# NeSC-IV/sage-icp

Measured on AMD Instinct MI355X. Metric: ICP frames/sec (120k-pt scan vs 1M-pt map), higher is better.
Workload: dtype f64

## Files before the change

profiles/loop_tail.py:

```python
import ctypes as C
import os
import sys

sys.path.insert(0, os.getcwd())
import numpy as np
import sage_icp_amd as sage

sage.LIB_PATH = os.environ.get("LOOP_LIB", os.path.join(os.path.dirname(sage.LIB_PATH), "_probe", "libsageicp_looptiming.so"))
from sage_icp_amd import synthetic as syn

div = int(sys.argv[1]) if len(sys.argv) > 1 else 1
p = syn.PARAMS[sys.argv[2] if len(sys.argv) > 2 else "cold"]
name = sys.argv[3] if len(sys.argv) > 3 else "c2"
w = syn.make_workload(name, lambda: sage.VoxelHashMap(syn.WORKLOADS[name]["voxel"], 100.0))
n = len(w["scan"]) // div
f = sage.Frame(w["map"], w["scan"][:n])
os.environ["SAGEICP_LOOP"] = "2"
sage.set_counting(False)
for _ in range(3):
    pose, st = sage.register_frame(f, w["map"], sage.IDENTITY, p["max_dist"], p["kernel"], p["sem_th"], return_stats=True)
assert st.single_launch == 1
IT, WG = 32, 2048
wg = np.zeros((IT, WG, 4), dtype=np.uint64)
sv = np.zeros((IT, 4), dtype=np.uint64)
# ... 46 lines not shown
    print("   %d CUs: " % len(keys) + "; ".join("%d hold %d workgroups (last counted in %.2f)" % ((pop == k).sum(), k, fin[pop[inv] == k].max()) for k in sorted(set(pop))))
    print("   extra units per CU: " + "; ".join("%d CUs with %d (last counted in %.2f)" % ((nx == k).sum(), k, fin[nx[inv] == k].max()) for k in sorted(set(nx))))
    late = np.argsort(-fin)[:10]
    print("   last ten: " + "; ".join("%.1f (%s, %d pts max, %d stale, %d pts, CU pop %d / %d extra)" % (
        fin[o], "extra %.1f-%.1f" % (s2[o], e2[o]) if extra[o] else "no extra", info[it, used, 1][o], info[it, used, 2][o], info[it, used, 3][o],
        pop[inv[o]], nx[inv[o]]) for o in late))

if hasattr(sage.lib(), "sageicp_debug_loop_waves"):
    wv = np.zeros((IT, WG, 8, 2), dtype=np.uint64)
    sage.lib().sageicp_debug_loop_waves(wv.ctypes.data_as(C.c_void_p))
    for it in (12,):
        if it >= min(IT, st.iterations):
            continue
        t0 = sv[it - 1, 3]
        rec = wv[it][used]
        nwv = int((rec[0, :, 0] > 0).sum())
        end = rec[:, :nwv, 0].astype(np.float64) / 100.0 - t0
        meta = rec[:, :nwv, 1]
        start = ((rec[:, :nwv, 0] & ~np.uint64((1 << 40) - 1)) | (meta >> np.uint64(24))).astype(np.float64) / 100.0 - t0
        unit = ((meta >> np.uint64(16)) & np.uint64(0xFF)).astype(int)
        simd = ((meta >> np.uint64(4)) & np.uint64(3)).astype(int)
        slot = (meta & np.uint64(0xF)).astype(int)
        print("iteration %d, first units of the %d waves of a workgroup:" % (it, nwv))
        for k in range(nwv):
            print("   wave %d: SIMD histogram %s | slot histogram %s | unit taken histogram %s | start p50 %.2f | end p10 %.2f p50 %.2f p90 %.2f p100 %.2f"
                  % (k, np.bincount(simd[:, k], minlength=4).tolist(), np.bincount(slot[:, k], minlength=10).tolist(),
                     np.bincount(unit[:, k], minlength=nwv).tolist(), np.median(start[:, k]), q(end[:, k], .1), q(end[:, k], .5), q(end[:, k], .9), end[:, k].max()))
        for u in range(nwv):
            sel = unit == u
            print("   unit %d (by last iteration's work, heaviest first): lasts p10 %.2f p50 %.2f p90 %.2f p100 %.2f | ends p50 %.2f p90 %.2f p100 %.2f"
                  % (u, q((end - start)[sel], .1), q((end - start)[sel], .5), q((end - start)[sel], .9), (end - start)[sel].max(),
                     q(end[sel], .5), q(end[sel], .9), end[sel].max()))
        print("   distinct SIMDs per workgroup: " + str(np.bincount([len(set(r)) for r in simd.tolist()], minlength=5).tolist()))
        xcc = (info[it, used, 0] >> 28).astype(np.int64)
        cu = ((info[it, used, 0] >> 8) & 0xF).astype(np.int64)
        se = ((info[it, used, 0] >> 13) & 0x7).astype(np.int64)
        key = (((xcc << 4 | se) << 4 | cu)[:, None] << 2) | simd
        keys, inv = np.unique(key.ravel(), return_inverse=True)
        heavy = np.zeros(len(keys)); cnt = np.zeros(len(keys)); last = np.zeros(len(keys))
        np.add.at(heavy, inv, (unit.ravel() == 0).astype(float))
        np.add.at(cnt, inv, 1.0)
        np.maximum.at(last, inv, end.ravel())
        print("   %d SIMDs: waves per SIMD histogram %s; heaviest units (unit 0) per SIMD histogram %s" % (len(keys), np.bincount(cnt.astype(int)).tolist(), np.bincount(heavy.astype(int)).tolist()))
        for h in sorted(set(heavy.astype(int))):
            print("      SIMDs with %d heaviest units: %d, last first-unit ends mean %.2f max %.2f" % (h, (heavy == h).sum(), last[heavy == h].mean(), last[heavy == h].max()))
```

sage-icp_amd/csrc/icp_body.h:

```cpp
#pragma once

namespace sageicp {

#ifndef SAGE_LOOP_FLAT_MINW
#define SAGE_LOOP_FLAT_MINW 8
#endif
#ifndef SAGE_SCAN_AHEAD
#define SAGE_SCAN_AHEAD 1
#endif
#ifndef SAGE_ROW_SHIFT_LAYER
#define SAGE_ROW_SHIFT_LAYER 1
#endif
#ifndef SAGE_ROW_SHIFT_MAXW
#define SAGE_ROW_SHIFT_MAXW 4
#endif

struct PairCompact {
    uint4 a, b;
    unsigned ka, oa;
    bool ha, hb;
};
struct PairFull {
    Point4 a, b;
    unsigned ka;
// ... 36 lines not shown
    const double slack = (GIVEN ? fs : 1e-9 * vs) + 1e-13 * fabs(v);
    const double lo = fmax((v - below_hi) - slack, 0.0);
    const double hi = fmax((above_lo - v) - slack, 0.0);
    g[0] = (lo * lo) * sc;
    g[1] = 0.0;
    g[2] = (hi * hi) * sc;
}

__device__ __forceinline__ float round_up_f32(double x) {
    return __uint_as_float(__float_as_uint(static_cast<float>(x)) + 1u);
}

template <int LW>
__device__ __forceinline__ bool reduce_argmin(double best, unsigned bkey, bool valid, const uint32_t *lrow, unsigned &mkey, unsigned &woff) {
    constexpr int W = 1 << LW, SH = 5;
    const double m = seg_min_f64<W>(best);
    const unsigned mine = (best == m) ? bkey : 0xFFFFFFFFu;
    mkey = seg_min_u32<W>(mine);
    const bool found = valid && mkey != 0xFFFFFFFFu;
    woff = (lrow[found ? mkey >> 8 : 0u] >> 8) * (kUnitPoints * 32u) + ((mkey & 255u) << SH);
    return found;
}

template <int LW, bool FUSED, bool FILT, bool PERSIST = false, bool FLATQ = false>
__device__ __forceinline__ void icp_body(const IcpParams &P, uint32_t *smem, LoopGroup *G = nullptr, const double *pose = nullptr) {
    static_assert(!PERSIST || FUSED, "the persistent loop always accumulates");
    constexpr int W = 1 << LW;
    constexpr int QW = 64 >> LW;
    constexpr int SH = 5;
    PROBE_NN_BEGIN(np);
    PROBE_DELAY_BEGIN(t0);
    int lane;
    if constexpr (PERSIST) {
        unsigned l;
        asm volatile("v_mbcnt_lo_u32_b32 %0, -1, 0\n\tv_mbcnt_hi_u32_b32 %0, -1, %0" : "=v"(l));
        lane = static_cast<int>(l);
    } else {
        lane = static_cast<int>(threadIdx.x & 63u);
    }
    const int wv = __builtin_amdgcn_readfirstlane(static_cast<int>(threadIdx.x >> 6));
    if (FUSED && !PERSIST) {
        if (threadIdx.x == 0) {
            smem[kWgArrive] = 0u;
            smem[kWgGo] = 0u;
        }
        if (threadIdx.x < 2u * kWgAccWords) smem[kWgAcc + threadIdx.x] = 0u;
        if (threadIdx.x < 12u && !(P.chain && P.chain_iter > 0))
            reinterpret_cast<double *>(smem + kWgPose)[threadIdx.x] = threadIdx.x < 9u ? P.st->R[threadIdx.x] : P.st->T[4u + threadIdx.x - 9u];
        __syncthreads();
    }
    uint32_t *wl;
    if constexpr (PERSIST) wl = G->rows;
    else wl = smem + kWgHeaderWords + static_cast<unsigned>(wv) * icp_wave_words(LW);

    unsigned wave_id, stripe_id = 0u;
    if constexpr (PERSIST) wave_id = G->slot;
    else wave_id = icp_wave_of_stripe(P, wv, stripe_id);

    const int qw = lane >> LW;
    const unsigned ci = static_cast<unsigned>(lane) & (W - 1u);
    unsigned q, qslot = 0u, bslot = 0u;
    if constexpr (PERSIST) {
        bslot = G->perm[G->unit * (QW / 4) + static_cast<unsigned>(qw >> 2)];
        qslot = bslot * 4u + (static_cast<unsigned>(qw) & 3u);
        q = G->q_first + qslot;
    } else {
        q = wave_id * QW + static_cast<unsigned>(qw);
    }
    const bool valid = q < static_cast<unsigned>(P.n);
    const unsigned qc = valid ? q : 0u;
    uint32_t *lrow = wl + (PERSIST ? qslot : static_cast<unsigned>(qw)) * kRowLdsStride;
    const uint32_t *grow = P.rows + static_cast<size_t>(qc) * kRowWords;

    const __amdgpu_buffer_rsrc_t pts = __builtin_amdgcn_make_buffer_rsrc(
        const_cast<Point4 *>(P.pts), 0, static_cast<int>(P.pts_bytes), 0x00020000);

    const __amdgpu_buffer_rsrc_t cands = __builtin_amdgcn_make_buffer_rsrc(
        const_cast<uint4 *>(P.cand), 0, static_cast<int>(P.cand_bytes), 0x00020000);
    constexpr int SHC = FILT ? 4 : 5;

    constexpr int NP = (7 + W - 1) / W;
    uint4 rk;
    uint2 prev = make_uint2(0xFFFFFFFFu, 0u);
    Point4 f;
    uint4 pc0 = make_uint4(0u, 0u, 0u, 0u), pc1 = pc0, pc2 = pc0, pc3 = pc0, pc4 = pc0, pc5 = pc0, pc6 = pc0;
    uint32_t *lst = nullptr;
    if constexpr (PERSIST) {
        lst = G->state + qslot * kLoopStateWords;
        const uint4 fa = *reinterpret_cast<const uint4 *>(lst), fb = *reinterpret_cast<const uint4 *>(lst + 4);
        const uint4 pk = *reinterpret_cast<const uint4 *>(lst + kStPrev);
        const uint2 ko = *reinterpret_cast<const uint2 *>(lst + kStPrev + 4);
        f.x = __hiloint2double(static_cast<int>(fa.y), static_cast<int>(fa.x));
        f.y = __hiloint2double(static_cast<int>(fa.w), static_cast<int>(fa.z));
        f.z = __hiloint2double(static_cast<int>(fb.y), static_cast<int>(fb.x));
        f.l = __hiloint2double(static_cast<int>(fb.w), static_cast<int>(fb.z));
        prev = make_uint2(pk.x, pk.y);
        rk = make_uint4(pk.z, pk.w, ko.x, ko.y);
    } else {
        rk = *reinterpret_cast<const uint4 *>(grow + kRowKey);
        if (FUSED) prev = P.nn_prev[qc];
        f = P.frame[qc];
        auto row_piece = [&](int k) {
            const unsigned p = min(ci + static_cast<unsigned>(W * k), 6u);
            return *reinterpret_cast<const uint4 *>(grow + 4u * p);
        };
        pc0 = row_piece(0); pc1 = pc0; pc2 = pc0; pc3 = pc0; pc4 = pc0; pc5 = pc0; pc6 = pc0;
        if (NP > 1) pc1 = row_piece(1);
        if (NP > 2) pc2 = row_piece(2);
        if (NP > 3) pc3 = row_piece(3);
        if (NP > 4) pc4 = row_piece(4);
        if (NP > 5) pc5 = row_piece(5);
        if (NP > 6) pc6 = row_piece(6);
    }
    PROBE_DELAY_WAIT(P, t0);
    if constexpr (FUSED && !PERSIST) {
        if (P.chain && P.chain_iter > 0) {
            if (wv == 0) chain_wait_pose(P, smem, lane);
            __syncthreads();
            if (smem[kWgGo]) return;
        }
    }
    const Query s = [&]() {
        if constexpr (PERSIST) {
            return make_query<(W >= 4)>(f, pose, pose + 9, 1, P.voxel_size, P.inv_voxel_size, static_cast<unsigned>(lane));
        } else if constexpr (FUSED) {
            const double *lpose = reinterpret_cast<const double *>(smem + kWgPose);
            return make_query<(W >= 4)>(f, lpose, lpose + 9, P.apply_pose, P.voxel_size, P.inv_voxel_size, threadIdx.x);
        } else {
            return make_query<(W >= 4)>(f, P.st->R, P.st->T + 4, P.apply_pose, P.voxel_size, P.inv_voxel_size, threadIdx.x);
        }
    }();
    const bool stale = valid && (static_cast<uint32_t>(s.kx) != rk.x || static_cast<uint32_t>(s.ky) != rk.y ||
                                 static_cast<uint32_t>(s.kz) != rk.z);
    unsigned occ = rk.w;
    NN_T(np, 0);
    LP_T(PERSIST, G, 0);
    if constexpr (!PERSIST) {
        auto stage = [&](int k, const uint4 &v) {
            const unsigned p = ci + static_cast<unsigned>(W * k);
            if (p < 7u) *reinterpret_cast<uint4 *>(lrow + 4u * p) = v;
        };
        stage(0, pc0);
        if (NP > 1) stage(1, pc1);
        if (NP > 2) stage(2, pc2);
// ... 156 lines not shown
            }
        }
    }
    if constexpr (PERSIST) {
        __builtin_amdgcn_fence(__ATOMIC_ACQ_REL, "wavefront");
        prev.x = lst[opaque_v(kStPrev)];
    }
    if (!valid) occ = 0u;

    double gx[3], gy[3], gz[3];
    {
        const double vs = P.voxel_size, sc = P.prune_scale;
        double fs = 0.0;
        if constexpr (PERSIST) fs = reinterpret_cast<const LoopArgs *>(&P)->face_slack;
        axis_gaps<PERSIST>(s.x, s.kx, vs, sc, fs, gx);
        axis_gaps<PERSIST>(s.y, s.ky, vs, sc, fs, gy);
        axis_gaps<PERSIST>(s.z, s.kz, vs, sc, fs, gz);
    }
    NN_T(np, 1);
    LP_T(PERSIST, G, 1);

    double best = P.dist_init;
    unsigned bkey = 0xFFFFFFFFu;
    const int pli = static_cast<int>(s.l);
    const double th = P.sem_th;
    unsigned npairs = 0u;

    unsigned k = ci, kend = 0u, off = 0u;
    unsigned pk = 0u, needs = 0u, wn = 0u;
    auto evaluate = [&](const Point4 &nb, bool on, unsigned key) {
        const double dx = nb.x - s.x, dy = nb.y - s.y, dz = nb.z - s.z;
        double d = SAGE_SQNORM3_NN(dx * dx, dy * dy, dz * dz);
        const bool same = static_cast<int>(nb.l) == pli || fabs(nb.l * s.l) < 1.0;
        const double ds = d * th;
        d = same ? ds : d;
        d = __hiloint2double(on ? __double2hiint(d) : 0x7FF80000, __double2loint(d));
        const bool lt = d < best, eq = d == best, kl = key < bkey;
        const bool take = lt | (eq & kl);
        best = min_f64(best, d);
        bkey = take ? key : bkey;
    };

    const float qx = static_cast<float>(s.x), qy = static_cast<float>(s.y), qz = static_cast<float>(s.z);
    const float plab = static_cast<float>(pli);
    const bool q_zero = pli == 0;
    bool unknown = false;
    double slack = 0.0;
// ... 177 lines not shown

    constexpr unsigned kHome = 13u;
    bool merged = false;
    if constexpr (PERSIST) {
        const bool seeded = valid && prev.x != 0xFFFFFFFFu;
        const Point4 pp = *reinterpret_cast<const Point4 *>(lst + 8);
        evaluate(pp, seeded, prev.x);
        merged = seeded;
        const unsigned first = seeded ? 0u : (occ & (1u << kHome));
        if (__ballot(first != 0u)) scan(first, nullptr, false, 0u);
    } else if (FUSED) {
        const bool seeded = valid && prev.x != 0xFFFFFFFFu;
        const Point4 pp = load_point(pts, seeded ? prev.y : 0u);
        scan(occ & (1u << kHome), &pp, seeded, prev.x);
    } else {
        scan(occ & (1u << kHome), nullptr, false, 0u);
    }
    NN_T(np, 2);
    LP_T(PERSIST, G, 2);
    const double bound = seg_min_f64<W>(best);
    fb = bound;
    unsigned need = P.keep_all;
    if constexpr (W >= 4) {
        const unsigned a = ci & 3u;
        const double ga = a == 0u ? gx[0] : (a == 2u ? gx[2] : 0.0);
        unsigned layer = 0u;
#pragma unroll
        for (int b = 0; b < 3; ++b) {
#pragma unroll
            for (int c = 0; c < 3; ++c) {
                const double lb = ga + (gy[b] + gz[c]);
                layer |= (lb <= bound) ? (1u << (3 * b + c)) : 0u;
            }
        }
        layer = (a < 3u && ci < 4u) ? layer << (9u * a) : 0u;
        layer |= dpp_u32<kDppXor1>(layer);
        layer |= dpp_u32<kDppXor2>(layer);
        if (W >= 8) layer |= dpp_u32<kDppHalfMirror>(layer);
        if (W >= 16) layer |= dpp_u32<kDppMirror>(layer);
        need |= layer & ~(1u << kHome);
    } else {
#pragma unroll
        for (int v = 0; v < 27; ++v) {
            if (v == static_cast<int>(kHome)) continue;
            const double lb = gx[v / 9] + (gy[(v / 3) % 3] + gz[v % 3]);
            need |= (lb <= bound) ? (1u << v) : 0u;
        }
// ... 129 lines not shown
```

sage-icp_amd/csrc/kernels.hip:

```cpp

#include <hip/hip_runtime.h>

#include <algorithm>
#include <cfloat>
#include <cstdlib>
#include <type_traits>
#include <vector>

#ifndef SAGE_ICP_STRIPE
#define SAGE_ICP_STRIPE 8
#endif
#ifndef SAGE_ICP_OCC
#define SAGE_ICP_OCC 6
#endif

#include "kernels.h"
#include "se3_math.h"
#include "sageicp_types.h"
#include "probes.h"

namespace sageicp {


template <int CTRL>
// ... 330 lines not shown
        {
            if (ok) (void)__hip_atomic_fetch_add(dst + lane, x, __ATOMIC_RELAXED, __HIP_MEMORY_SCOPE_AGENT);
            else (void)__hip_atomic_fetch_or(overflow, 1ll, __ATOMIC_RELAXED, __HIP_MEMORY_SCOPE_AGENT);
        }
    }
}

struct LoopGroup {
    uint32_t *rows;
    uint32_t *state;
    const uint32_t *perm;
    uint32_t *work;
    unsigned unit;
    double *red;
    unsigned long long *wgacc;
    unsigned q_first;
    unsigned slot;
    PROBE_LOOP_GROUP_FIELDS
};
constexpr int kLoopMaxWaves = kLoopMaxWavesHost;
constexpr unsigned kLoopStripe = kLoopStripeHost;
constexpr int kNoVoxel = 0x7FFFFFFF;
constexpr unsigned kStPrev = 16, kStKey = 18;
constexpr unsigned kLpArrive = 0, kLpNext = 1, kLpDone = 2;
constexpr unsigned kLpPose = 4;
constexpr unsigned kLpDbg = kLpPose + 24u;
constexpr unsigned kLpFirst = kLpDbg + 4u;
constexpr unsigned kLpAcc = kLpFirst + 8u;
constexpr unsigned kLpHeaderWords = (kLpAcc + 2u * kWgAccWords + 15u) & ~15u;
__host__ __device__ constexpr unsigned loop_red_words() { return 2u * kCount * 4u; }
__host__ __device__ constexpr unsigned loop_perm_words(unsigned nblk) { return 2u * ((nblk + 7u) & ~7u); }
template <typename W>
struct LoopLds {
    W perm, work, rows, state, red, end;
    __host__ __device__ constexpr LoopLds(int lw, W nw, W gpw)
        : perm(kLpHeaderWords),
          work(perm + loop_perm_words(static_cast<unsigned>(gpw) * ((64u >> lw) / 4u)) / 2u),
          rows(perm + loop_perm_words(static_cast<unsigned>(gpw) * ((64u >> lw) / 4u))),
          state(rows + gpw * static_cast<W>(64 >> lw) * static_cast<W>(kRowLdsStride)),
          red(state + gpw * static_cast<W>(64 >> lw) * static_cast<W>(kLoopStateWords)),
          end(red + nw * loop_red_words()) {}
};

__device__ __forceinline__ unsigned loop_pose_copy(int pose_map, unsigned b = blockIdx.x) {
    return pose_map == 1 ? 0u : ((pose_map == 2 ? b + 3u : b) & static_cast<unsigned>(kLoopPoseCopies - 1));
}
__device__ __forceinline__ void chain_wait_pose(const IcpParams &P, uint32_t *smem, int lane) {
// ... 304 lines not shown
```

sage-icp_amd/csrc/loop_kernel.h:

```cpp
#pragma once

namespace sageicp {


__device__ __forceinline__ int exchange_sums_wave(double *S, const P2pParams &X, unsigned long long g) {
    const int lane = static_cast<int>(threadIdx.x & 63u);
    const int slot = static_cast<int>(g & 1ull);
    const unsigned long long tag = g + 1ull;
    if (lane < kNumSums) {
        const double v = S[lane];
        for (int r = 0; r < X.nranks; ++r)
            __hip_atomic_store(&X.block[r]->sums[slot][X.rank][lane], v, __ATOMIC_RELAXED, __HIP_MEMORY_SCOPE_SYSTEM);
    }
    asm volatile("s_waitcnt vmcnt(0)" ::: "memory");
    __builtin_amdgcn_fence(__ATOMIC_RELEASE, "");
    asm volatile("s_waitcnt vmcnt(0)" ::: "memory");
    if (lane == 0)
        for (int r = 0; r < X.nranks; ++r)
            __hip_atomic_store(&X.block[r]->flag[X.rank], tag, __ATOMIC_RELAXED, __HIP_MEMORY_SCOPE_SYSTEM);
    P2pBlock *mine = X.block[X.rank];
    bool late = false, gone = false;
    if (lane < X.nranks) {
        const unsigned long long t0 = __builtin_amdgcn_s_memrealtime();
        while (__hip_atomic_load(&mine->flag[lane], __ATOMIC_RELAXED, __HIP_MEMORY_SCOPE_SYSTEM) < tag) {
// ... 296 lines not shown
            idx = jb;
            nwg = static_cast<unsigned>(L.wgs) >> 3;
        } else {
            idx = ((jb / kLoopStripe) * 8u + xcd) * kLoopStripe + (jb % kLoopStripe);
            nwg = static_cast<unsigned>(L.wgs);
        }
        const unsigned base = cnt / nwg, extra = cnt - base * nwg;
        g0 = lo + idx * base + min(idx, extra);
        gcnt = min(gpw, base + (idx < extra ? 1u : 0u));
    }
    constexpr unsigned BPW = QW / 4;
    const unsigned nblk_max = gpw * BPW;
    const LoopLds<unsigned> lds0(LW, static_cast<unsigned>(nw), gpw);
    uint32_t *perm0 = smem + lds0.perm;
    uint32_t *work0 = smem + lds0.work;
    uint32_t *state0 = smem + lds0.state;

    if (threadIdx.x < 9) s_pose[threadIdx.x] = P.st->R[threadIdx.x];
    else if (threadIdx.x < 12) s_pose[threadIdx.x] = P.st->T[4 + threadIdx.x - 9];
    if (threadIdx.x == 0) {
        smem[kLpArrive] = 0u;
        smem[kLpNext] = 0u;
        smem[kLpDone] = 0u;
        PROBE_LOOP_CLEAR_STATS(smem);
    }
    if (L.deal && (threadIdx.x & 63u) == 0u) {
        unsigned hw;
        asm volatile("s_getreg_b32 %0, hwreg(HW_REG_HW_ID)" : "=s"(hw));
        smem[kLpFirst + static_cast<unsigned>(wv)] = (((hw >> 4) & 3u) + (hw & 15u)) % static_cast<unsigned>(nw);
    }
    for (unsigned i = threadIdx.x; i < 2u * kWgAccWords; i += blockDim.x) smem[kLpAcc + i] = 0u;
    for (unsigned i = threadIdx.x; i < nblk_max; i += blockDim.x) {
        perm0[i] = i;
        work0[i] = 0u;
    }
    for (unsigned sl = threadIdx.x; sl < gcnt * QW; sl += blockDim.x) {
        const unsigned q = g0 * QW + sl;
        const Point4 f = P.frame[q < static_cast<unsigned>(P.n) ? q : 0u];
        {
            uint32_t *lst = state0 + sl * kLoopStateWords;
            *reinterpret_cast<Point4 *>(lst) = f;
            Point4 z;
            z.x = z.y = z.z = z.l = 0.0;
            *reinterpret_cast<Point4 *>(lst + 8) = z;
            *reinterpret_cast<uint4 *>(lst + kStPrev) = make_uint4(0xFFFFFFFFu, 0u, static_cast<uint32_t>(kNoVoxel),
                                                                   static_cast<uint32_t>(kNoVoxel));
// ... 6 lines not shown
        for (int w2 = 0; w2 < nw; ++w2) {
            const unsigned pr = smem[kLpFirst + static_cast<unsigned>(w2)];
            table[w2] = pr;
            if (!((claimed >> pr) & 1u)) { claimed |= 1u << pr; kept |= 1u << w2; }
        }
        for (int w2 = 0; w2 < nw; ++w2)
            if (!((kept >> w2) & 1u)) {
                const unsigned pr = static_cast<unsigned>(__builtin_ctz(~claimed));
                table[w2] = pr;
                claimed |= 1u << pr;
            }
        __syncthreads();
        if (threadIdx.x == 0) {
            for (int w2 = 0; w2 < nw; ++w2) smem[kLpFirst + static_cast<unsigned>(w2)] = table[w2];
            smem[kLpNext] = static_cast<unsigned>(nw);
        }
        __syncthreads();
    }
    static_assert(kLoopMaxWaves <= 8, "k_loop keeps the wave's index in three bits");
    const unsigned who = (blockIdx.x << 3) | static_cast<unsigned>(wv);
    PROBE_LOOP_BEGIN(lp);


    for (int it = 0;; ++it) {
        auto ka = __builtin_amdgcn_kernarg_segment_ptr();
        asm volatile("" : "+s"(ka));
        bool dealt = ((const LoopArgs *)(ka))->L.deal != 0;
        for (;;) {
            unsigned gi = 0u;
            if (dealt) {
                dealt = false;
                gi = static_cast<unsigned>(__builtin_amdgcn_readfirstlane(static_cast<int>(smem[kLpFirst + (opaque_s(who) & 7u)])));
                if (gi >= opaque_s(gcnt)) continue;
            } else {
                if (lane_now() == 0)
                    gi = __hip_atomic_fetch_add(&smem[kLpNext], 1u, __ATOMIC_RELAXED, __HIP_MEMORY_SCOPE_WORKGROUP);
                gi = static_cast<unsigned>(__builtin_amdgcn_readfirstlane(static_cast<int>(gi)));
                if (gi >= opaque_s(gcnt)) break;
            }
            auto kb = __builtin_amdgcn_kernarg_segment_ptr();
            asm volatile("" : "+s"(kb));
            const LoopArgs &B = *(const LoopArgs *)(kb);
            if (B.L.prio) loop_set_priority(gi, B.L.nw, B.L.prio);
            PROBE_LOOP_UNIT_BEGIN(it, gi, B.L.nw, t_unit);
            const LoopLds<unsigned> lds(LW, static_cast<unsigned>(B.L.nw), static_cast<unsigned>(B.L.gpw));
            const unsigned first = opaque_s(g0);
            LoopGroup G;
            G.rows = smem + lds.rows;
            G.state = smem + lds.state;
            G.perm = smem + lds.perm;
            G.work = smem + lds.work;
            G.unit = gi;
            G.red = reinterpret_cast<double *>(smem + lds.red + (opaque_s(who) & 7u) * loop_red_words());
            G.wgacc = reinterpret_cast<unsigned long long *>(smem + kLpAcc);
            G.q_first = first * QW;
            G.slot = first + gi;
            PROBE_LOOP_PASS_BEGIN(lp, G);
            icp_body<LW, true, FILT, true>(B.P, smem, &G, s_pose);
            PROBE_LOOP_UNIT_END(lp, G, it, gi, B.L.nw, static_cast<int>(opaque_s(who) & 7u), lane_now(), t_unit);
        }
        PROBE_LOOP_MARK(t_a);
        auto kc = __builtin_amdgcn_kernarg_segment_ptr();
        asm volatile("" : "+s"(kc));
        const LoopParams &L = ((const LoopArgs *)(kc))->L;
        LoopShared *sh = L.sh;
        const int lane = lane_now();
        const unsigned me = opaque_s(who), wg = me >> 3;
        unsigned prior = 0u;
        __atomic_signal_fence(__ATOMIC_SEQ_CST);
        if (lane == 0)
            prior = __hip_atomic_fetch_add(&smem[kLpArrive], 1u, __ATOMIC_RELAXED, __HIP_MEMORY_SCOPE_WORKGROUP);
        __atomic_signal_fence(__ATOMIC_SEQ_CST);
        prior = static_cast<unsigned>(__builtin_amdgcn_readfirstlane(static_cast<int>(prior)));
        const bool last = prior == static_cast<unsigned>(L.nw) - 1u;
        if (last) {
            wgacc_flush<true, true>(reinterpret_cast<unsigned long long *>(smem + kLpAcc), &sh->acc[it & 1][wg & (kLoopReplicas - 1)][0],
                                    &sh->acc[it & 1][0][kAccWords - 1]);
            if (lane == 0) {
                smem[kLpArrive] = 0u;
                smem[kLpNext] = L.deal ? static_cast<unsigned>(L.nw) : 0u;
            }
            const unsigned nblk = opaque_s(gcnt) * BPW;
            if (nblk <= 64u && nblk > BPW) {
                const LoopLds<unsigned> lds(LW, static_cast<unsigned>(L.nw), static_cast<unsigned>(L.gpw));
                uint32_t *perm = smem + lds.perm, *work = smem + lds.work;
                __builtin_amdgcn_fence(__ATOMIC_ACQ_REL, "wavefront");
                const unsigned i = static_cast<unsigned>(lane);
                const unsigned wi = i < nblk ? work[i] : 0u;
                unsigned rank = 0u;
                for (unsigned j = 0; j < nblk; ++j) {
                    const unsigned wj = work[j];
                    rank += (wj > wi || (wj == wi && j < i)) ? 1u : 0u;
                }
                __builtin_amdgcn_fence(__ATOMIC_ACQ_REL, "wavefront");
                if (i < nblk) {
                    perm[rank] = i;
                    work[i] = 0u;
                }
            }
            PROBE_LOOP_WG_INFO(smem, it, lane);
            LOOP_STAMP_WG(it, 0);
        }
        if ((me & 7u) == 0u) {
            const unsigned long long tag = static_cast<unsigned long long>(it) + 1ull;
            const unsigned long long t0 = __builtin_amdgcn_s_memrealtime();
            unsigned long long g = tag << 32;
            bool aborted = false;
            for (;;) {
                if (lane < kLoopPoseGranules) g = ld_agent(&sh->pose[loop_pose_copy(L.pose_map, wg)][lane]);
                const bool ok = (g >> 32) == tag;
                if (__all(ok)) break;
                unsigned long long ab = 0ull;
                if (lane == 0) ab = ld_agent(&sh->abort_word[0]);
                const bool late = __builtin_amdgcn_s_memrealtime() - t0 > L.timeout_ticks;
                if (__any(ab != 0ull) || late) {
                    if (lane == 0 && late) {
                        st_agent(&sh->abort_word[0], 1ull);
                        L.st->loop_aborted = 1;
                    }
                    aborted = true;
                    break;
                }
                __builtin_amdgcn_s_sleep(SAGE_LOOP_POLL_SLEEP);
                if (L.wgs > 1024) __builtin_amdgcn_s_sleep(SAGE_LOOP_POLL_SLEEP);
            }
            if (aborted) {
                if (lane == 0) smem[kLpDone] = 2u;
            } else {
                if (lane < 24) reinterpret_cast<uint32_t *>(s_pose)[lane] = static_cast<uint32_t>(g);
                if (lane == 24) smem[kLpDone] = static_cast<uint32_t>(g);
            }
            LOOP_STAMP_WG(it, 1);
        }
        PROBE_LOOP_CLOSED(lp, last, t_a, t_b);
        __syncthreads();
        PROBE_LOOP_WAITED(lp, t_b);
        if (smem[kLpDone]) break;
    }
    PROBE_LOOP_END(lp);
}

}
```

sage-icp_amd/csrc/probes.h:

```cpp
#pragma once

#include <algorithm>
#include <vector>

namespace sageicp {

#ifdef SAGE_NN_TIMING
constexpr unsigned kNnTimingSlots = 1u << 17;
__device__ unsigned long long g_nn_phase[8ull * kNnTimingSlots];
__device__ unsigned long long g_nn_span[4ull * kNnTimingSlots];
__device__ int g_nn_span_iter;
struct NnProbe {
    unsigned long long tph[5] = {0, 0, 0, 0, 0};
    unsigned long long tprev = __builtin_amdgcn_s_memtime();
    unsigned long long tstart = tprev;
    unsigned long long rstart = __builtin_amdgcn_s_memrealtime();
    unsigned n_consume = 0u, n_exact = 0u, n_exact_lanes = 0u;
};
#define PROBE_NN_BEGIN(np) NnProbe np
#define NN_T(np, i) do { const unsigned long long _t = __builtin_amdgcn_s_memtime(); (np).tph[i] += _t - (np).tprev; (np).tprev = _t; } while (0)
#define PROBE_NN_CONSUME(np) ++(np).n_consume
#define PROBE_NN_EXACT(np, pa, pb) do { ++(np).n_exact; (np).n_exact_lanes += static_cast<unsigned>(__popcll(__ballot(pa)) + __popcll(__ballot(pb))); } while (0)
#define PROBE_NN_WORK(P, q, first_lane, npairs) do { if ((first_lane) && (P).work) (P).work[q] = (npairs); } while (0)
#define PROBE_NN_END(np, P, valid, ci, npairs, lane, wave_id)                                                              \
// ... 40 lines not shown
    for (int i = 0; i < 16; ++i) out[i] = 0;
    for (unsigned s = 0; s < kNnTimingSlots; ++s) {
        const unsigned long long *t = &h[8ull * s];
        if (!t[7]) continue;
        for (int k = 0; k < 8; ++k) out[k] += t[k];
        if (t[5] / t[7] > out[8]) out[8] = t[5] / t[7];
        ++out[9];
    }
    if (reset) {
        std::fill(h.begin(), h.end(), 0ull);
        (void)hipMemcpyToSymbol(HIP_SYMBOL(g_nn_phase), h.data(), h.size() * sizeof(unsigned long long));
    }
}
#else
#define NN_T(np, i) do { } while (0)
#define PROBE_NN_BEGIN(np) do { } while (0)
#define PROBE_NN_CONSUME(np) do { } while (0)
#define PROBE_NN_EXACT(np, pa, pb) do { } while (0)
#define PROBE_NN_WORK(P, q, first_lane, npairs) do { } while (0)
#define PROBE_NN_END(np, P, valid, ci, npairs, lane, wave_id) do { } while (0)
#endif

#ifdef SAGE_LOOP_TIMING
#define PROBE_LOOP_GROUP_FIELDS unsigned long long ph[8], tprev;
#define LP_T(persist, G, i) do { if constexpr (persist) { const unsigned long long _t = __builtin_amdgcn_s_memtime(); (G)->ph[i] += _t - (G)->tprev; (G)->tprev = _t; } } while (0)
#define PROBE_LOOP_WAVE_STATS(smem, valid, ci, npairs, stale, lane)                                                        \
    do {                                                                                                                   \
        unsigned mx = (valid) ? (npairs) : 0u, sm = ((valid) && (ci) == 0u) ? (npairs) : 0u, stl = ((stale) && (ci) == 0u) ? 1u : 0u; \
        for (int d = 1; d < 64; d <<= 1) {                                                                                 \
            mx = max(mx, static_cast<unsigned>(__shfl_xor(mx, d, 64)));                                                    \
            sm += __shfl_xor(sm, d, 64);                                                                                   \
            stl += __shfl_xor(stl, d, 64);                                                                                 \
        }                                                                                                                  \
        if ((lane) == 0) {                                                                                                 \
            atomicMax(&(smem)[kLpDbg], mx);                                                                                \
            atomicAdd(&(smem)[kLpDbg + 1], stl);                                                                           \
            atomicAdd(&(smem)[kLpDbg + 2], sm);                                                                            \
        }                                                                                                                  \
    } while (0)
constexpr int kLoopTimedIters = 32, kLoopTimedWgs = 2048;
__device__ unsigned long long g_loop_wg[kLoopTimedIters][kLoopTimedWgs][4];
__device__ unsigned g_loop_wginfo[kLoopTimedIters][kLoopTimedWgs][4];
__device__ unsigned long long g_loop_solver[kLoopTimedIters][4];
__device__ unsigned long long g_loop_solver2[kLoopTimedIters][4];
__device__ unsigned long long g_loop_wave[kLoopTimedIters][kLoopTimedWgs][8][2];
__device__ unsigned long long g_loop_phase[16];
#define LOOP_STAMP_SOLVER(it, k) do { if ((it) < kLoopTimedIters && (threadIdx.x & 63u) == 0u) g_loop_solver[it][k] = __builtin_amdgcn_s_memrealtime(); } while (0)
#define LOOP_STAMP_SOLVER2(it, k) do { if ((it) < kLoopTimedIters && (threadIdx.x & 63u) == 0u) g_loop_solver2[it][k] = __builtin_amdgcn_s_memrealtime(); } while (0)
#define LOOP_STAMP_WG(it, k) do { if ((it) < kLoopTimedIters && blockIdx.x < kLoopTimedWgs && (threadIdx.x & 63u) == 0u) g_loop_wg[it][blockIdx.x][k] = __builtin_amdgcn_s_memrealtime(); } while (0)
#define PROBE_LOOP_BEGIN(lp)                                                                                               \
    unsigned long long lp##_ph[8] = {0, 0, 0, 0, 0, 0, 0, 0};                                                              \
    unsigned long long lp##_t_wait = 0, lp##_t_close = 0, lp##_n_pass = 0
#define PROBE_LOOP_CLEAR_STATS(smem) { (smem)[kLpDbg] = 0u; (smem)[kLpDbg + 1] = 0u; (smem)[kLpDbg + 2] = 0u; }
#define PROBE_LOOP_UNIT_BEGIN(it, gi, nw, t_unit)                                                                          \
    if ((gi) >= static_cast<unsigned>(nw)) LOOP_STAMP_WG(it, 2);                                                           \
    const unsigned long long t_unit = __builtin_amdgcn_s_memrealtime()
#define PROBE_LOOP_PASS_BEGIN(lp, G)                                                                                       \
    {                                                                                                                      \
        for (int i = 0; i < 8; ++i) (G).ph[i] = 0;                                                                         \
        (G).tprev = __builtin_amdgcn_s_memtime();                                                                          \
        ++lp##_n_pass;                                                                                                     \
    }
#define PROBE_LOOP_UNIT_END(lp, G, it, gi, nw, wv, lane, t_unit)                                                           \
    {                                                                                                                      \
        if ((gi) >= static_cast<unsigned>(nw)) LOOP_STAMP_WG(it, 3);                                                       \
        if ((it) < kLoopTimedIters && blockIdx.x < kLoopTimedWgs && (lane) == 0 && (wv) < 8 && (gi) < static_cast<unsigned>(nw)) { \
            unsigned hw;                                                                                                   \
            asm volatile("s_getreg_b32 %0, hwreg(HW_REG_HW_ID)" : "=s"(hw));                                               \
            g_loop_wave[it][blockIdx.x][wv][0] = __builtin_amdgcn_s_memrealtime();                                         \
            g_loop_wave[it][blockIdx.x][wv][1] = ((t_unit) << 24) | (static_cast<unsigned long long>((gi) & 0xFFu) << 16) | (hw & 0xFFFFu); \
        }                                                                                                                  \
        for (int i = 0; i < 8; ++i) lp##_ph[i] += (G).ph[i];                                                               \
    }
#define PROBE_LOOP_MARK(t) const unsigned long long t = __builtin_amdgcn_s_memtime()
#define PROBE_LOOP_WG_INFO(smem, it, lane)                                                                                 \
    {                                                                                                                      \
        if ((lane) == 0 && (it) < kLoopTimedIters && blockIdx.x < kLoopTimedWgs) {                                         \
            unsigned hw;                                                                                                   \
            asm volatile("s_getreg_b32 %0, hwreg(HW_REG_HW_ID)" : "=s"(hw));                                               \
            unsigned xcc;                                                                                                  \
            asm volatile("s_getreg_b32 %0, hwreg(HW_REG_XCC_ID)" : "=s"(xcc));                                             \
            unsigned *o = g_loop_wginfo[it][blockIdx.x];                                                                   \
            o[0] = (xcc << 28) | (hw & 0x0FFFFFFFu);                                                                       \
            o[1] = (smem)[kLpDbg]; o[2] = (smem)[kLpDbg + 1]; o[3] = (smem)[kLpDbg + 2];                                   \
            (smem)[kLpDbg] = 0u; (smem)[kLpDbg + 1] = 0u; (smem)[kLpDbg + 2] = 0u;                                         \
        }                                                                                                                  \
    }
#define PROBE_LOOP_CLOSED(lp, last, t_a, t_b)                                                                              \
    const unsigned long long t_b = __builtin_amdgcn_s_memtime();                                                           \
    if (last) lp##_t_close += t_b - (t_a)
#define PROBE_LOOP_WAITED(lp, t_b) lp##_t_wait += __builtin_amdgcn_s_memtime() - (t_b)
#define PROBE_LOOP_END(lp)                                                                                                 \
    {                                                                                                                      \
        if ((threadIdx.x & 63u) == 0u) {                                                                                   \
            for (int i = 0; i < 8; ++i) atomicAdd(&g_loop_phase[i], lp##_ph[i]);                                           \
            atomicAdd(&g_loop_phase[8], lp##_t_wait);                                                                      \
            atomicAdd(&g_loop_phase[9], lp##_t_close);                                                                     \
            atomicAdd(&g_loop_phase[10], lp##_n_pass);                                                                     \
        }                                                                                                                  \
    }
extern "C" void sageicp_debug_loop_solver2(unsigned long long *out) {
    (void)hipMemcpyFromSymbol(out, HIP_SYMBOL(g_loop_solver2), sizeof(unsigned long long) * kLoopTimedIters * 4);
}
extern "C" void sageicp_debug_loop_phases(unsigned long long *out, int reset) {
    (void)hipMemcpyFromSymbol(out, HIP_SYMBOL(g_loop_phase), sizeof(unsigned long long) * 16);
    if (reset) {
        unsigned long long z[16] = {0};
        (void)hipMemcpyToSymbol(HIP_SYMBOL(g_loop_phase), z, sizeof(z));
    }
}
extern "C" void sageicp_debug_loop_waves(unsigned long long *out) {
    (void)hipMemcpyFromSymbol(out, HIP_SYMBOL(g_loop_wave), sizeof(unsigned long long) * kLoopTimedIters * kLoopTimedWgs * 8 * 2);
}
extern "C" void sageicp_debug_loop_info(unsigned *info) {
    (void)hipMemcpyFromSymbol(info, HIP_SYMBOL(g_loop_wginfo), sizeof(unsigned) * kLoopTimedIters * kLoopTimedWgs * 4);
}
extern "C" void sageicp_debug_loop_times(unsigned long long *wg, unsigned long long *solver) {
    (void)hipMemcpyFromSymbol(wg, HIP_SYMBOL(g_loop_wg), sizeof(unsigned long long) * kLoopTimedIters * kLoopTimedWgs * 4);
    (void)hipMemcpyFromSymbol(solver, HIP_SYMBOL(g_loop_solver), sizeof(unsigned long long) * kLoopTimedIters * 4);
}
#else
#define LP_T(persist, G, i) do { } while (0)
#define PROBE_LOOP_GROUP_FIELDS
#define LOOP_STAMP_SOLVER(it, k) do { } while (0)
#define LOOP_STAMP_SOLVER2(it, k) do { } while (0)
#define LOOP_STAMP_WG(it, k) do { } while (0)
#define PROBE_LOOP_BEGIN(lp) ((void)0)
#define PROBE_LOOP_CLEAR_STATS(smem) ((void)0)
#define PROBE_LOOP_UNIT_BEGIN(it, gi, nw, t_unit) ((void)0)
#define PROBE_LOOP_PASS_BEGIN(lp, G) ((void)0)
#define PROBE_LOOP_UNIT_END(lp, G, it, gi, nw, wv, lane, t_unit) ((void)0)
#define PROBE_LOOP_MARK(t) ((void)0)
#define PROBE_LOOP_WG_INFO(smem, it, lane) ((void)0)
#define PROBE_LOOP_CLOSED(lp, last, t_a, t_b) ((void)0)
#define PROBE_LOOP_WAITED(lp, t_b) ((void)0)
#define PROBE_LOOP_END(lp) ((void)0)
#define PROBE_LOOP_WAVE_STATS(smem, valid, ci, npairs, stale, lane) do { } while (0)
#endif

#ifdef SAGE_GN_TIMING
__device__ unsigned long long g_gn_phase[16];
#define PROBE_FIN_START(t_start) const unsigned long long t_start = __builtin_amdgcn_s_memrealtime()
#define PROBE_FIN_REDUCED(t_start) do { if (threadIdx.x == 0) atomicAdd(&g_gn_phase[8], __builtin_amdgcn_s_memrealtime() - (t_start)); } while (0)
#define PROBE_FIN_BEGIN(ft) unsigned long long ft[8]
#define FIN_STAMP(ft, i) do { if (threadIdx.x == 0) (ft)[i] = __builtin_amdgcn_s_memrealtime(); } while (0)
#define PROBE_FIN_END(ft)                                                                                                  \
    do {                                                                                                                   \
        (ft)[4] = __builtin_amdgcn_s_memrealtime();                                                                        \
        for (int i = 1; i < 4; ++i) atomicAdd(&g_gn_phase[8 + i], (ft)[i + 1] - (ft)[i]);                                  \
        atomicAdd(&g_gn_phase[4], 1ull);                                                                                   \
    } while (0)
extern "C" void sageicp_debug_gn_phases(unsigned long long out[16], int reset) {
    (void)hipMemcpyFromSymbol(out, HIP_SYMBOL(g_gn_phase), sizeof(unsigned long long) * 16);
    if (reset) {
        unsigned long long z[16] = {0};
        (void)hipMemcpyToSymbol(HIP_SYMBOL(g_gn_phase), z, sizeof(z));
    }
// ... 34 lines not shown
```

Measured before the change: 245.2.

## Stage pose-independent query state before waiting for the iteration pose

Splits the persistent-loop ICP body into two halves. The first half loads a wave's first unit (permutation slot, stored point, previous neighbour key and row keys) before the workgroup polls for the new pose. The second half runs the pose-dependent search after the barrier. The pose wait moves to the top of the loop, with an iteration counter kept in LDS, so the state loads overlap the cross-workgroup pose latency. This adds live registers for the staged state, reorders the loop's barrier structure, and adds timing probes that measure pose-to-first-use latency.

```diff
diff --git a/profiles/loop_tail.py b/profiles/loop_tail.py
--- a/profiles/loop_tail.py
+++ b/profiles/loop_tail.py
@@ -92,6 +92,17 @@
         simd = ((meta >> np.uint64(4)) & np.uint64(3)).astype(int)
         slot = (meta & np.uint64(0xF)).astype(int)
         print("iteration %d, first units of the %d waves of a workgroup:" % (it, nwv))
+        if hasattr(sage.lib(), "sageicp_debug_loop_wave_pose"):
+            wp = np.zeros((IT, WG, 8), dtype=np.uint64)
+            sage.lib().sageicp_debug_loop_wave_pose(wp.ctypes.data_as(C.c_void_p))
+            for jt in (6, 12, 20):
+                if jt >= min(IT, st.iterations):
+                    continue
+                use = wp[jt][used][:, :nwv].astype(np.float64) / 100.0
+                heldw = wg[jt - 1, used, 1][:, None]
+                hop = (use - heldw)[(wv[jt][used][:, :nwv, 0] > 0) & (use > 0)]
+                print("   iteration %d: pose held by the workgroup -> first pose-dependent instruction of a wave's first pass: p10 %.2f p50 %.2f p90 %.2f p99 %.2f p100 %.2f us (%d waves)"
+                      % (jt, q(hop, .1), q(hop, .5), q(hop, .9), q(hop, .99), hop.max(), hop.size))
         for k in range(nwv):
             print("   wave %d: SIMD histogram %s | slot histogram %s | unit taken histogram %s | start p50 %.2f | end p10 %.2f p50 %.2f p90 %.2f p100 %.2f"
                   % (k, np.bincount(simd[:, k], minlength=4).tolist(), np.bincount(slot[:, k], minlength=10).tolist(),
diff --git a/sage-icp_amd/csrc/icp_body.h b/sage-icp_amd/csrc/icp_body.h
--- a/sage-icp_amd/csrc/icp_body.h
+++ b/sage-icp_amd/csrc/icp_body.h
@@ -82,9 +82,19 @@
     return found;
 }
 
-template <int LW, bool FUSED, bool FILT, bool PERSIST = false, bool FLATQ = false>
-__device__ __forceinline__ void icp_body(const IcpParams &P, uint32_t *smem, LoopGroup *G = nullptr, const double *pose = nullptr) {
+struct LoopStaged {
+    unsigned qslot;
+    double fx, fy, fz, fl;
+    unsigned prev_key, prev_off;
+    unsigned kx, ky, kz, occ;
+    int pli;
+};
+
+template <int LW, bool FUSED, bool FILT, bool PERSIST = false, bool FLATQ = false, int HALF = 0>
+__device__ __forceinline__ void icp_body(const IcpParams &P, uint32_t *smem, LoopGroup *G = nullptr, const double *pose = nullptr,
+                                         LoopStaged *S = nullptr) {
     static_assert(!PERSIST || FUSED, "the persistent loop always accumulates");
+    static_assert(PERSIST ? (HALF == 1 || HALF == 2) : HALF == 0, "k_loop runs the pass in two halves, k_icp in one");
     constexpr int W = 1 << LW;
     constexpr int QW = 64 >> LW;
     constexpr int SH = 5;
@@ -121,8 +131,12 @@
     const unsigned ci = static_cast<unsigned>(lane) & (W - 1u);
     unsigned q, qslot = 0u, bslot = 0u;
     if constexpr (PERSIST) {
-        bslot = G->perm[G->unit * (QW / 4) + static_cast<unsigned>(qw >> 2)];
-        qslot = bslot * 4u + (static_cast<unsigned>(qw) & 3u);
+        if constexpr (HALF == 1) {
+            bslot = G->perm[G->unit * (QW / 4) + static_cast<unsigned>(qw >> 2)];
+            qslot = bslot * 4u + (static_cast<unsigned>(qw) & 3u);
+        } else {
+            qslot = S->qslot;
+        }
         q = G->q_first + qslot;
     } else {
         q = wave_id * QW + static_cast<unsigned>(qw);
@@ -147,15 +161,23 @@
     uint32_t *lst = nullptr;
     if constexpr (PERSIST) {
         lst = G->state + qslot * kLoopStateWords;
-        const uint4 fa = *reinterpret_cast<const uint4 *>(lst), fb = *reinterpret_cast<const uint4 *>(lst + 4);
-        const uint4 pk = *reinterpret_cast<const uint4 *>(lst + kStPrev);
-        const uint2 ko = *reinterpret_cast<const uint2 *>(lst + kStPrev + 4);
-        f.x = __hiloint2double(static_cast<int>(fa.y), static_cast<int>(fa.x));
-        f.y = __hiloint2double(static_cast<int>(fa.w), static_cast<int>(fa.z));
-        f.z = __hiloint2double(static_cast<int>(fb.y), static_cast<int>(fb.x));
-        f.l = __hiloint2double(static_cast<int>(fb.w), static_cast<int>(fb.z));
-        prev = make_uint2(pk.x, pk.y);
-        rk = make_uint4(pk.z, pk.w, ko.x, ko.y);
+        if constexpr (HALF == 1) {
+            const uint4 fa = *reinterpret_cast<const uint4 *>(lst), fb = *reinterpret_cast<const uint4 *>(lst + 4);
+            const uint4 pk = *reinterpret_cast<const uint4 *>(lst + kStPrev);
+            const uint2 ko = *reinterpret_cast<const uint2 *>(lst + kStPrev + 4);
+            S->qslot = qslot;
+            S->fx = __hiloint2double(static_cast<int>(fa.y), static_cast<int>(fa.x));
+            S->fy = __hiloint2double(static_cast<int>(fa.w), static_cast<int>(fa.z));
+            S->fz = __hiloint2double(static_cast<int>(fb.y), static_cast<int>(fb.x));
+            S->fl = __hiloint2double(static_cast<int>(fb.w), static_cast<int>(fb.z));
+            S->prev_key = pk.x; S->prev_off = pk.y;
+            S->kx = pk.z; S->ky = pk.w; S->kz = ko.x; S->occ = ko.y;
+            S->pli = static_cast<int>(S->fl);
+            return;
+        }
+        f.x = S->fx; f.y = S->fy; f.z = S->fz; f.l = S->fl;
+        prev = make_uint2(S->prev_key, S->prev_off);
+        rk = make_uint4(S->kx, S->ky, S->kz, S->occ);
     } else {
         rk = *reinterpret_cast<const uint4 *>(grow + kRowKey);
         if (FUSED) prev = P.nn_prev[qc];
@@ -180,6 +202,7 @@
             if (smem[kWgGo]) return;
         }
     }
+    PROBE_LOOP_POSE_USE(PERSIST, G);
     const Query s = [&]() {
         if constexpr (PERSIST) {
             return make_query<(W >= 4)>(f, pose, pose + 9, 1, P.voxel_size, P.inv_voxel_size, static_cast<unsigned>(lane));
@@ -382,7 +405,7 @@
 
     double best = P.dist_init;
     unsigned bkey = 0xFFFFFFFFu;
-    const int pli = static_cast<int>(s.l);
+    const int pli = HALF == 2 ? S->pli : static_cast<int>(s.l);
     const double th = P.sem_th;
     unsigned npairs = 0u;
 
@@ -606,7 +629,7 @@
     fb = bound;
     unsigned need = P.keep_all;
     if constexpr (W >= 4) {
-        const unsigned a = ci & 3u;
+        const unsigned a = (PERSIST ? static_cast<unsigned>(lane_now()) : ci) & 3u;
         const double ga = a == 0u ? gx[0] : (a == 2u ? gx[2] : 0.0);
         unsigned layer = 0u;
 #pragma unroll
diff --git a/sage-icp_amd/csrc/kernels.hip b/sage-icp_amd/csrc/kernels.hip
--- a/sage-icp_amd/csrc/kernels.hip
+++ b/sage-icp_amd/csrc/kernels.hip
@@ -376,7 +376,7 @@
 constexpr unsigned kLoopStripe = kLoopStripeHost;
 constexpr int kNoVoxel = 0x7FFFFFFF;
 constexpr unsigned kStPrev = 16, kStKey = 18;
-constexpr unsigned kLpArrive = 0, kLpNext = 1, kLpDone = 2;
+constexpr unsigned kLpArrive = 0, kLpNext = 1, kLpDone = 2, kLpIter = 3;
 constexpr unsigned kLpPose = 4;
 constexpr unsigned kLpDbg = kLpPose + 24u;
 constexpr unsigned kLpFirst = kLpDbg + 4u;
diff --git a/sage-icp_amd/csrc/loop_kernel.h b/sage-icp_amd/csrc/loop_kernel.h
--- a/sage-icp_amd/csrc/loop_kernel.h
+++ b/sage-icp_amd/csrc/loop_kernel.h
@@ -342,6 +342,7 @@
         smem[kLpArrive] = 0u;
         smem[kLpNext] = 0u;
         smem[kLpDone] = 0u;
+        smem[kLpIter] = 0u;
         PROBE_LOOP_CLEAR_STATS(smem);
     }
     if (L.deal && (threadIdx.x & 63u) == 0u) {
@@ -394,42 +395,101 @@
     PROBE_LOOP_BEGIN(lp);
 
 
-    for (int it = 0;; ++it) {
-        auto ka = __builtin_amdgcn_kernarg_segment_ptr();
-        asm volatile("" : "+s"(ka));
-        bool dealt = ((const LoopArgs *)(ka))->L.deal != 0;
-        for (;;) {
-            unsigned gi = 0u;
-            if (dealt) {
-                dealt = false;
-                gi = static_cast<unsigned>(__builtin_amdgcn_readfirstlane(static_cast<int>(smem[kLpFirst + (opaque_s(who) & 7u)])));
-                if (gi >= opaque_s(gcnt)) continue;
-            } else {
-                if (lane_now() == 0)
-                    gi = __hip_atomic_fetch_add(&smem[kLpNext], 1u, __ATOMIC_RELAXED, __HIP_MEMORY_SCOPE_WORKGROUP);
-                gi = static_cast<unsigned>(__builtin_amdgcn_readfirstlane(static_cast<int>(gi)));
-                if (gi >= opaque_s(gcnt)) break;
-            }
-            auto kb = __builtin_amdgcn_kernarg_segment_ptr();
-            asm volatile("" : "+s"(kb));
-            const LoopArgs &B = *(const LoopArgs *)(kb);
-            if (B.L.prio) loop_set_priority(gi, B.L.nw, B.L.prio);
-            PROBE_LOOP_UNIT_BEGIN(it, gi, B.L.nw, t_unit);
+    for (;;) {
+        PROBE_LOOP_IT(it, smem);
+        constexpr unsigned kNoUnit = 0xFFFFFFFFu;
+        LoopStaged S{};
+        PROBE_LOOP_UNIT_VAR(t_unit);
+        auto group_of = [&](unsigned u, const LoopArgs &B) {
             const LoopLds<unsigned> lds(LW, static_cast<unsigned>(B.L.nw), static_cast<unsigned>(B.L.gpw));
-            const unsigned first = opaque_s(g0);
+            const unsigned first_unit = opaque_s(g0);
             LoopGroup G;
             G.rows = smem + lds.rows;
             G.state = smem + lds.state;
             G.perm = smem + lds.perm;
             G.work = smem + lds.work;
-            G.unit = gi;
+            G.unit = u;
             G.red = reinterpret_cast<double *>(smem + lds.red + (opaque_s(who) & 7u) * loop_red_words());
             G.wgacc = reinterpret_cast<unsigned long long *>(smem + kLpAcc);
-            G.q_first = first * QW;
-            G.slot = first + gi;
-            PROBE_LOOP_PASS_BEGIN(lp, G);
-            icp_body<LW, true, FILT, true>(B.P, smem, &G, s_pose);
-            PROBE_LOOP_UNIT_END(lp, G, it, gi, B.L.nw, static_cast<int>(opaque_s(who) & 7u), lane_now(), t_unit);
+            G.q_first = first_unit * QW;
+            G.slot = first_unit + u;
+            return G;
+        };
+        auto stage = [&](unsigned u) {
+            auto kb = __builtin_amdgcn_kernarg_segment_ptr();
+            asm volatile("" : "+s"(kb));
+            const LoopArgs &B = *(const LoopArgs *)(kb);
+            if (B.L.prio) loop_set_priority(u, B.L.nw, B.L.prio);
+            PROBE_LOOP_UNIT_BEGIN(it, u, B.L.nw, t_unit);
+            LoopGroup G = group_of(u, B);
+            icp_body<LW, true, FILT, true, false, 1>(B.P, smem, &G, nullptr, &S);
+        };
+        auto ka = __builtin_amdgcn_kernarg_segment_ptr();
+        asm volatile("" : "+s"(ka));
+        unsigned gi = kNoUnit;
+        if (((const LoopArgs *)(ka))->L.deal) {
+            gi = static_cast<unsigned>(__builtin_amdgcn_readfirstlane(static_cast<int>(smem[kLpFirst + (opaque_s(who) & 7u)])));
+            if (gi >= opaque_s(gcnt)) gi = kNoUnit;
+        }
+        if (gi != kNoUnit) stage(gi);
+        {
+            const LoopParams &L = ((const LoopArgs *)(ka))->L;
+            const unsigned itn = (opaque_s(who) & 7u) == 0u ? static_cast<unsigned>(__builtin_amdgcn_readfirstlane(static_cast<int>(smem[kLpIter]))) : 0u;
+            if (itn != 0u) {
+                LoopShared *sh = L.sh;
+                const int lane = lane_now();
+                const unsigned wg = opaque_s(who) >> 3;
+                const unsigned long long tag = static_cast<unsigned long long>(itn);
+                const unsigned long long t0 = __builtin_amdgcn_s_memrealtime();
+                unsigned long long g = tag << 32;
+                bool aborted = false;
+                for (;;) {
+                    if (lane < kLoopPoseGranules) g = ld_agent(&sh->pose[loop_pose_copy(L.pose_map, wg)][lane]);
+                    const bool ok = (g >> 32) == tag;
+                    if (__all(ok)) break;
+                    unsigned long long ab = 0ull;
+                    if (lane == 0) ab = ld_agent(&sh->abort_word[0]);
+                    const bool late = __builtin_amdgcn_s_memrealtime() - t0 > L.timeout_ticks;
+                    if (__any(ab != 0ull) || late) {
+                        if (lane == 0 && late) {
+                            st_agent(&sh->abort_word[0], 1ull);
+                            L.st->loop_aborted = 1;
+                        }
+                        aborted = true;
+                        break;
+                    }
+                    __builtin_amdgcn_s_sleep(SAGE_LOOP_POLL_SLEEP);
+                    if (L.wgs > 1024) __builtin_amdgcn_s_sleep(SAGE_LOOP_POLL_SLEEP);
+                }
+                if (aborted) {
+                    if (lane == 0) smem[kLpDone] = 2u;
+                } else {
+                    if (lane < 24) smem[kLpPose + static_cast<unsigned>(lane)] = static_cast<uint32_t>(g);
+                    if (lane == 24) smem[kLpDone] = static_cast<uint32_t>(g);
+                }
+                LOOP_STAMP_WG(itn - 1u, 1);
+            }
+        }
+        PROBE_LOOP_WAIT_BEGIN(t_b);
+        __syncthreads();
+        PROBE_LOOP_WAITED(lp, t_b);
+        if (smem[kLpDone]) break;
+        for (;;) {
+            if (gi != kNoUnit) {
+                auto kb = __builtin_amdgcn_kernarg_segment_ptr();
+                asm volatile("" : "+s"(kb));
+                const LoopArgs &B = *(const LoopArgs *)(kb);
+                LoopGroup G = group_of(opaque_s(gi), B);
+                PROBE_LOOP_PASS_BEGIN(lp, G);
+                icp_body<LW, true, FILT, true, false, 2>(B.P, smem, &G, reinterpret_cast<const double *>(smem + kLpPose), &S);
+                PROBE_LOOP_UNIT_END(lp, G, it, gi, B.L.nw, static_cast<int>(opaque_s(who) & 7u), lane_now(), t_unit);
+            }
+            gi = 0u;
+            if (lane_now() == 0)
+                gi = __hip_atomic_fetch_add(&smem[kLpNext], 1u, __ATOMIC_RELAXED, __HIP_MEMORY_SCOPE_WORKGROUP);
+            gi = static_cast<unsigned>(__builtin_amdgcn_readfirstlane(static_cast<int>(gi)));
+            if (gi >= opaque_s(gcnt)) break;
+            stage(gi);
         }
         PROBE_LOOP_MARK(t_a);
         auto kc = __builtin_amdgcn_kernarg_segment_ptr();
@@ -446,10 +506,12 @@
         prior = static_cast<unsigned>(__builtin_amdgcn_readfirstlane(static_cast<int>(prior)));
         const bool last = prior == static_cast<unsigned>(L.nw) - 1u;
         if (last) {
+            const int it = __builtin_amdgcn_readfirstlane(static_cast<int>(smem[kLpIter]));
             wgacc_flush<true, true>(reinterpret_cast<unsigned long long *>(smem + kLpAcc), &sh->acc[it & 1][wg & (kLoopReplicas - 1)][0],
                                     &sh->acc[it & 1][0][kAccWords - 1]);
             if (lane == 0) {
                 smem[kLpArrive] = 0u;
+                smem[kLpIter] = static_cast<unsigned>(it) + 1u;
                 smem[kLpNext] = L.deal ? static_cast<unsigned>(L.nw) : 0u;
             }
             const unsigned nblk = opaque_s(gcnt) * BPW;
@@ -473,41 +535,10 @@
             PROBE_LOOP_WG_INFO(smem, it, lane);
             LOOP_STAMP_WG(it, 0);
         }
-        if ((me & 7u) == 0u) {
-            const unsigned long long tag = static_cast<unsigned long long>(it) + 1ull;
-            const unsigned long long t0 = __builtin_amdgcn_s_memrealtime();
-            unsigned long long g = tag << 32;
-            bool aborted = false;
-            for (;;) {
-                if (lane < kLoopPoseGranules) g = ld_agent(&sh->pose[loop_pose_copy(L.pose_map, wg)][lane]);
-                const bool ok = (g >> 32) == tag;
-                if (__all(ok)) break;
-                unsigned long long ab = 0ull;
-                if (lane == 0) ab = ld_agent(&sh->abort_word[0]);
-                const bool late = __builtin_amdgcn_s_memrealtime() - t0 > L.timeout_ticks;
-                if (__any(ab != 0ull) || late) {
-                    if (lane == 0 && late) {
-                        st_agent(&sh->abort_word[0], 1ull);
-                        L.st->loop_aborted = 1;
-                    }
-                    aborted = true;
-                    break;
-                }
-                __builtin_amdgcn_s_sleep(SAGE_LOOP_POLL_SLEEP);
-                if (L.wgs > 1024) __builtin_amdgcn_s_sleep(SAGE_LOOP_POLL_SLEEP);
-            }
-            if (aborted) {
-                if (lane == 0) smem[kLpDone] = 2u;
-            } else {
-                if (lane < 24) reinterpret_cast<uint32_t *>(s_pose)[lane] = static_cast<uint32_t>(g);
-                if (lane == 24) smem[kLpDone] = static_cast<uint32_t>(g);
-            }
-            LOOP_STAMP_WG(it, 1);
-        }
-        PROBE_LOOP_CLOSED(lp, last, t_a, t_b);
+        PROBE_LOOP_CLOSED(lp, last, t_a);
+        PROBE_LOOP_WAIT_BEGIN(t_c);
         __syncthreads();
-        PROBE_LOOP_WAITED(lp, t_b);
-        if (smem[kLpDone]) break;
+        PROBE_LOOP_WAITED(lp, t_c);
     }
     PROBE_LOOP_END(lp);
 }
diff --git a/sage-icp_amd/csrc/probes.h b/sage-icp_amd/csrc/probes.h
--- a/sage-icp_amd/csrc/probes.h
+++ b/sage-icp_amd/csrc/probes.h
@@ -86,7 +86,8 @@
 #endif
 
 #ifdef SAGE_LOOP_TIMING
-#define PROBE_LOOP_GROUP_FIELDS unsigned long long ph[8], tprev;
+#define PROBE_LOOP_GROUP_FIELDS unsigned long long ph[8], tprev, tpose;
+#define PROBE_LOOP_POSE_USE(persist, G) do { if constexpr (persist) (G)->tpose = __builtin_amdgcn_s_memrealtime(); } while (0)
 #define LP_T(persist, G, i) do { if constexpr (persist) { const unsigned long long _t = __builtin_amdgcn_s_memtime(); (G)->ph[i] += _t - (G)->tprev; (G)->tprev = _t; } } while (0)
 #define PROBE_LOOP_WAVE_STATS(smem, valid, ci, npairs, stale, lane)                                                        \
     do {                                                                                                                   \
@@ -108,6 +109,7 @@
 __device__ unsigned long long g_loop_solver[kLoopTimedIters][4];
 __device__ unsigned long long g_loop_solver2[kLoopTimedIters][4];
 __device__ unsigned long long g_loop_wave[kLoopTimedIters][kLoopTimedWgs][8][2];
+__device__ unsigned long long g_loop_wave_pose[kLoopTimedIters][kLoopTimedWgs][8];
 __device__ unsigned long long g_loop_phase[16];
 #define LOOP_STAMP_SOLVER(it, k) do { if ((it) < kLoopTimedIters && (threadIdx.x & 63u) == 0u) g_loop_solver[it][k] = __builtin_amdgcn_s_memrealtime(); } while (0)
 #define LOOP_STAMP_SOLVER2(it, k) do { if ((it) < kLoopTimedIters && (threadIdx.x & 63u) == 0u) g_loop_solver2[it][k] = __builtin_amdgcn_s_memrealtime(); } while (0)
@@ -116,9 +118,11 @@
     unsigned long long lp##_ph[8] = {0, 0, 0, 0, 0, 0, 0, 0};                                                              \
     unsigned long long lp##_t_wait = 0, lp##_t_close = 0, lp##_n_pass = 0
 #define PROBE_LOOP_CLEAR_STATS(smem) { (smem)[kLpDbg] = 0u; (smem)[kLpDbg + 1] = 0u; (smem)[kLpDbg + 2] = 0u; }
+#define PROBE_LOOP_IT(it, smem) const int it = __builtin_amdgcn_readfirstlane(static_cast<int>((smem)[kLpIter]))
+#define PROBE_LOOP_UNIT_VAR(t_unit) unsigned long long t_unit = 0
 #define PROBE_LOOP_UNIT_BEGIN(it, gi, nw, t_unit)                                                                          \
     if ((gi) >= static_cast<unsigned>(nw)) LOOP_STAMP_WG(it, 2);                                                           \
-    const unsigned long long t_unit = __builtin_amdgcn_s_memrealtime()
+    t_unit = __builtin_amdgcn_s_memrealtime()
 #define PROBE_LOOP_PASS_BEGIN(lp, G)                                                                                       \
     {                                                                                                                      \
         for (int i = 0; i < 8; ++i) (G).ph[i] = 0;                                                                         \
@@ -133,6 +137,7 @@
             asm volatile("s_getreg_b32 %0, hwreg(HW_REG_HW_ID)" : "=s"(hw));                                               \
             g_loop_wave[it][blockIdx.x][wv][0] = __builtin_amdgcn_s_memrealtime();                                         \
             g_loop_wave[it][blockIdx.x][wv][1] = ((t_unit) << 24) | (static_cast<unsigned long long>((gi) & 0xFFu) << 16) | (hw & 0xFFFFu); \
+            g_loop_wave_pose[it][blockIdx.x][wv] = (G).tpose;                                                              \
         }                                                                                                                  \
         for (int i = 0; i < 8; ++i) lp##_ph[i] += (G).ph[i];                                                               \
     }
@@ -150,9 +155,9 @@
             (smem)[kLpDbg] = 0u; (smem)[kLpDbg + 1] = 0u; (smem)[kLpDbg + 2] = 0u;                                         \
         }                                                                                                                  \
     }
-#define PROBE_LOOP_CLOSED(lp, last, t_a, t_b)                                                                              \
-    const unsigned long long t_b = __builtin_amdgcn_s_memtime();                                                           \
-    if (last) lp##_t_close += t_b - (t_a)
+#define PROBE_LOOP_CLOSED(lp, last, t_a)                                                                                   \
+    if (last) lp##_t_close += __builtin_amdgcn_s_memtime() - (t_a)
+#define PROBE_LOOP_WAIT_BEGIN(t_b) const unsigned long long t_b = __builtin_amdgcn_s_memtime()
 #define PROBE_LOOP_WAITED(lp, t_b) lp##_t_wait += __builtin_amdgcn_s_memtime() - (t_b)
 #define PROBE_LOOP_END(lp)                                                                                                 \
     {                                                                                                                      \
@@ -175,6 +180,9 @@
 }
 extern "C" void sageicp_debug_loop_waves(unsigned long long *out) {
     (void)hipMemcpyFromSymbol(out, HIP_SYMBOL(g_loop_wave), sizeof(unsigned long long) * kLoopTimedIters * kLoopTimedWgs * 8 * 2);
+}
+extern "C" void sageicp_debug_loop_wave_pose(unsigned long long *out) {
+    (void)hipMemcpyFromSymbol(out, HIP_SYMBOL(g_loop_wave_pose), sizeof(unsigned long long) * kLoopTimedIters * kLoopTimedWgs * 8);
 }
 extern "C" void sageicp_debug_loop_info(unsigned *info) {
     (void)hipMemcpyFromSymbol(info, HIP_SYMBOL(g_loop_wginfo), sizeof(unsigned) * kLoopTimedIters * kLoopTimedWgs * 4);
@@ -191,12 +199,16 @@
 #define LOOP_STAMP_WG(it, k) do { } while (0)
 #define PROBE_LOOP_BEGIN(lp) ((void)0)
 #define PROBE_LOOP_CLEAR_STATS(smem) ((void)0)
+#define PROBE_LOOP_POSE_USE(persist, G) do { } while (0)
+#define PROBE_LOOP_UNIT_VAR(t_unit) ((void)0)
+#define PROBE_LOOP_IT(it, smem) ((void)0)
 #define PROBE_LOOP_UNIT_BEGIN(it, gi, nw, t_unit) ((void)0)
 #define PROBE_LOOP_PASS_BEGIN(lp, G) ((void)0)
 #define PROBE_LOOP_UNIT_END(lp, G, it, gi, nw, wv, lane, t_unit) ((void)0)
 #define PROBE_LOOP_MARK(t) ((void)0)
 #define PROBE_LOOP_WG_INFO(smem, it, lane) ((void)0)
-#define PROBE_LOOP_CLOSED(lp, last, t_a, t_b) ((void)0)
+#define PROBE_LOOP_CLOSED(lp, last, t_a) ((void)0)
+#define PROBE_LOOP_WAIT_BEGIN(t_b) ((void)0)
 #define PROBE_LOOP_WAITED(lp, t_b) ((void)0)
 #define PROBE_LOOP_END(lp) ((void)0)
 #define PROBE_LOOP_WAVE_STATS(smem, valid, ci, npairs, stale, lane) do { } while (0)
```

Result: faster. 248.6 (median of 6 runs) (+1.4%).
